# fulliu/lc

Measured on AMD Instinct MI355X. Metric: poses/sec (cov-loss fwd+bwd + weighted PnP), B=256 N=64, 1/2/4/8 MI355X, higher is better.
Workload: dtype f64; 1 GPU; configs[1]: synthetic B=256 N=64 2D-3D correspondences per GPU, HIP weighted-PnP + cov-loss; global_batch=256, n_points=64, launch=graph_region, launch_agreed_by_all_ranks=True

## Files before the change

### lc_amd/csrc/lc_common.h

```cpp
#pragma once
#include <hip/hip_runtime.h>

namespace lc {

#ifndef LC_NT_GRAD_STORES
#define LC_NT_GRAD_STORES 1
#endif
typedef float lc_v4f_t __attribute__((ext_vector_type(4)));
__device__ __forceinline__ void store_stream4(float* q, float a, float b, float c, float d) {
#if LC_NT_GRAD_STORES
    lc_v4f_t r = {a, b, c, d};
    __builtin_nontemporal_store(r, reinterpret_cast<lc_v4f_t*>(q));
#else
    *reinterpret_cast<float4*>(q) = make_float4(a, b, c, d);
#endif
}


constexpr int kWave = 64;

constexpr int kDppQuadXor1 = 0xB1;
constexpr int kDppQuadXor2 = 0x4E;
constexpr int kDppIdentity = 0xE4;
constexpr int kDppRowMirror = 0x140;
constexpr int kDppHalfMirror = 0x141;

template <int CTRL, int BANK_MASK = 0xF>
__device__ __forceinline__ double dpp_mov_f64(double old, double src) {
    const int lo = __builtin_amdgcn_update_dpp(__double2loint(old), __double2loint(src), CTRL, 0xF, BANK_MASK, false);
    const int hi = __builtin_amdgcn_update_dpp(__double2hiint(old), __double2hiint(src), CTRL, 0xF, BANK_MASK, false);
    return __hiloint2double(hi, lo);
}

__device__ __forceinline__ double shfl_f64(double v, int src) {
    const int lo = __shfl(__double2loint(v), src, kWave), hi = __shfl(__double2hiint(v), src, kWave);
    return __hiloint2double(hi, lo);
}

__device__ __forceinline__ double swap32_add(double a, double b) {
    const auto lo = __builtin_amdgcn_permlane32_swap(__double2loint(a), __double2loint(b), false, false);
    const auto hi = __builtin_amdgcn_permlane32_swap(__double2hiint(a), __double2hiint(b), false, false);
    return __hiloint2double(hi[0], lo[0]) + __hiloint2double(hi[1], lo[1]);
}
__device__ __forceinline__ double swap16_add(double a, double b) {
    const auto lo = __builtin_amdgcn_permlane16_swap(__double2loint(a), __double2loint(b), false, false);
    const auto hi = __builtin_amdgcn_permlane16_swap(__double2hiint(a), __double2hiint(b), false, false);
    return __hiloint2double(hi[0], lo[0]) + __hiloint2double(hi[1], lo[1]);
}

template <int CTRL, int BANK_UP>
__device__ __forceinline__ double dpp_exchange_add(double lo, double hi) {
    constexpr int BANK_DOWN = 0xF & ~BANK_UP;
    const double keep = dpp_mov_f64<kDppIdentity, BANK_UP>(lo, hi);
    double recv = dpp_mov_f64<CTRL, BANK_UP>(lo, hi);
    recv = dpp_mov_f64<CTRL, BANK_DOWN>(recv, lo);
    return keep + recv;
}

template <int K>
__device__ __forceinline__ void wave_allreduce(double (&v)[K]) {
#pragma unroll
    for (int i = 0; i < K; ++i) {
        double x = v[i];
        x += dpp_mov_f64<kDppQuadXor1>(x, x);
        x += dpp_mov_f64<kDppQuadXor2>(x, x);
        x += dpp_mov_f64<kDppHalfMirror>(x, x);
        x += dpp_mov_f64<kDppRowMirror>(x, x);
        x = swap16_add(x, x);
        x = swap32_add(x, x);
        v[i] = x;
    }
}

template <int K>
__device__ __forceinline__ void wave_reduce_scatter16(double (&v)[K], int ) {
    static_assert(K % 16 == 0, "K must be a multiple of 16");
    constexpr int R = K / 16;
#pragma unroll
    for (int i = 0; i < K / 2; ++i) v[i] = swap32_add(v[i], v[i + K / 2]);
#pragma unroll
    for (int i = 0; i < K / 4; ++i) v[i] = swap16_add(v[i], v[i + K / 4]);
#pragma unroll
    for (int i = 0; i < K / 8; ++i) v[i] = dpp_exchange_add<kDppRowMirror, 0xC>(v[i], v[i + K / 8]);
#pragma unroll
    for (int i = 0; i < K / 16; ++i) v[i] = dpp_exchange_add<kDppHalfMirror, 0xA>(v[i], v[i + K / 16]);
#pragma unroll
    for (int i = 0; i < R; ++i) {
        v[i] += dpp_mov_f64<kDppQuadXor2>(v[i], v[i]);
        v[i] += dpp_mov_f64<kDppQuadXor1>(v[i], v[i]);
    }
}

__device__ __forceinline__ int scatter16_base(int lane, int R) {
    return R * (((lane >> 5) & 1) * 8 + ((lane >> 4) & 1) * 4 + ((lane >> 3) & 1) * 2 + ((lane >> 2) & 1));
}

__device__ __forceinline__ double fast_rcp(double x) {
    const double y = __builtin_amdgcn_rcp(x);
    const double e = __builtin_fma(-x, y, 1.0);
    return __builtin_fma(y, e, y);
}

__device__ __forceinline__ void fast_sqrt_rsqrt(double x, double& s, double& rs) {
    const double r0 = __builtin_amdgcn_rsq(x);
    const double g = x * r0, h = 0.5 * r0;
    const double rr = __builtin_fma(-h, g, 0.5);
    const double g1 = __builtin_fma(g, rr, g), h1 = __builtin_fma(h, rr, h);
    s = x == 0.0 ? 0.0 : g1;
    rs = x == 0.0 ? r0 : 2.0 * h1;
}
__device__ __forceinline__ double fast_sqrt(double x) {
    double s, rs;
    fast_sqrt_rsqrt(x, s, rs);
    return s;
}

template <int NW>
constexpr int sum_bcast_lds_doubles(int K) { return K * 68 * NW + K; }

#ifndef LC_WAVE_SYNC
#define LC_WAVE_SYNC 0
#endif
__device__ __forceinline__ void wave_sync() {
    __builtin_amdgcn_fence(__ATOMIC_RELEASE, "wavefront");
    __builtin_amdgcn_wave_barrier();
    __builtin_amdgcn_fence(__ATOMIC_ACQUIRE, "wavefront");
}

template <class T>
__device__ __forceinline__ void xcd_store(T* q, T v) { __hip_atomic_store(q, v, __ATOMIC_RELAXED, __HIP_MEMORY_SCOPE_AGENT); }
template <class T>
__device__ __forceinline__ T xcd_load(const T* q) { return __hip_atomic_load(q, __ATOMIC_RELAXED, __HIP_MEMORY_SCOPE_AGENT); }
__device__ __forceinline__ void xcd_stores_done() { asm volatile("s_waitcnt vmcnt(0)" ::: "memory"); }

constexpr int kArrivalShards = 16, kArrivalStride = 32;
constexpr int kArrivalWords = (1 + kArrivalShards) * kArrivalStride;
__device__ __forceinline__ bool arrive_is_last(unsigned* words, unsigned block, unsigned blocks) {
    const unsigned shards = blocks < (unsigned)kArrivalShards ? blocks : (unsigned)kArrivalShards;
    const unsigned g = block % shards, members = (blocks - g + shards - 1) / shards;
    if (__hip_atomic_fetch_add(words + (1 + g) * kArrivalStride, 1u, __ATOMIC_RELAXED, __HIP_MEMORY_SCOPE_AGENT) != members - 1) return false;
    return __hip_atomic_fetch_add(words, 1u, __ATOMIC_RELAXED, __HIP_MEMORY_SCOPE_AGENT) == shards - 1;
}
__device__ __forceinline__ void arrival_reset(unsigned* words, int tid) {
    if (tid <= kArrivalShards) xcd_store(words + tid * kArrivalStride, 0u);
}

template <int NW>
__device__ __forceinline__ void block_sum_sync() {
    if constexpr (NW == 1 && !LC_WAVE_SYNC) wave_sync();
    else __syncthreads();
}

template <int NW>
__device__ __forceinline__ int block_sum_open(int tid) {
    block_sum_sync<NW>();
    return tid + 2 * (tid >> 5);
}
template <int NW>
__device__ __forceinline__ void block_sum_put(double* lds, int pos, int k, double v) { lds[k * (68 * NW) + pos] = v; }

template <int K, int NW>
__device__ __forceinline__ void block_sum_close(double (&v)[K], double* lds, int tid);

template <int K, int NW>
__device__ __forceinline__ void block_sum_bcast_lds(double (&v)[K], double* lds, int tid) {
    const int pos = block_sum_open<NW>(tid);
#pragma unroll
    for (int k = 0; k < K; ++k) block_sum_put<NW>(lds, pos, k, v[k]);
    block_sum_close<K, NW>(v, lds, tid);
}

template <int K, int NW>
__device__ __forceinline__ double* block_sum_totals(double* lds) { return lds + K * (68 * NW); }

template <int K, int NW>
__device__ __forceinline__ void block_sum_reduce(double* lds, int tid) {
    static_assert(K <= 32 && (NW == 1 || NW == 4), "unsupported shape");
    constexpr int LD = 68 * NW, S = 2 * NW;
    block_sum_sync<NW>();
    double s = 0;
    if (tid < K * S) {
        const double2* row = reinterpret_cast<const double2*>(lds + (tid / S) * LD + 34 * (tid % S));
        double2 a[8];
#pragma unroll
        for (int i = 0; i < 8; ++i) a[i] = row[i];
#pragma unroll
        for (int i = 0; i < 8; ++i) {
            const double2 t = row[8 + i];
            a[i].x += t.x;
            a[i].y += t.y;
        }
#pragma unroll
        for (int st = 4; st >= 1; st >>= 1) {
#pragma unroll
            for (int i = 0; i < st; ++i) { a[i].x += a[i + st].x; a[i].y += a[i + st].y; }
        }
        s = a[0].x + a[0].y;
    }
    s += dpp_mov_f64<kDppQuadXor1>(s, s);
    if constexpr (NW == 4) {
        s += dpp_mov_f64<kDppQuadXor2>(s, s);
        s += dpp_mov_f64<kDppHalfMirror>(s, s);
    }
    double* tot = lds + K * LD;
    if (tid < K * S && (tid % S) == 0) tot[tid / S] = s;
    block_sum_sync<NW>();
}

template <int K, int NW>
__device__ __forceinline__ void block_sum_close(double (&v)[K], double* lds, int tid) {
    block_sum_reduce<K, NW>(lds, tid);
    const double* tot = block_sum_totals<K, NW>(lds);
#pragma unroll
    for (int k = 0; k < K; ++k) v[k] = tot[k];
}

#ifndef LC_WIDE_SUM_REGS
#define LC_WIDE_SUM_REGS 1
#endif
template <int K>
__device__ __forceinline__ void block_sum_waves4(double (&v)[K], double* lds, int tid, int& phase) {
    static_assert(K <= 32, "one reduce-scatter of 32");
    const int lane = tid & 63, wave = tid >> 6;
    double w[32];
#pragma unroll
    for (int k = 0; k < 32; ++k) w[k] = k < K ? v[k] : 0.0;
    wave_reduce_scatter16<32>(w, lane);
    double* part = lds;
    double* tot = lds + 128 + 32 * phase;
    phase ^= 1;
    if ((lane & 3) == 0) *reinterpret_cast<double2*>(part + 32 * wave + scatter16_base(lane, 2)) = make_double2(w[0], w[1]);
    __syncthreads();
    if (tid < 32) tot[tid] = ((part[tid] + part[32 + tid]) + part[64 + tid]) + part[96 + tid];
    __syncthreads();
#pragma unroll
    for (int k = 0; k < K; ++k) v[k] = tot[k];
}

constexpr int kSplitMaxParts = 8;
#ifndef LC_SPLIT_WAIT_US
#define LC_SPLIT_WAIT_US 2000
#endif
constexpr unsigned long long kSplitWaitTicks = 100ull * LC_SPLIT_WAIT_US;
__device__ __forceinline__ bool split_wait_expired(int polls, unsigned long long& t0) {
    if ((polls & 15) != 15) return false;
    const unsigned long long now = __builtin_amdgcn_s_memrealtime();
    if (t0 == 0) { t0 = now; return false; }
    return now - t0 > kSplitWaitTicks;
}
constexpr int kSplitRowWords = 64;
constexpr size_t kSplitPoseBytes = 2 * kSplitMaxParts * kSplitRowWords * sizeof(unsigned long long) + 128;
constexpr int kSplitLdsDoubles = 128 + 64 + 2;
constexpr int kSplitSerialLdsDoubles = 128 + 32 * kSplitMaxParts + 32;
struct SplitSum {
    unsigned long long* exch;
    unsigned* epoch;
    int G, part;
    unsigned base;
    unsigned seq;
    bool timed_out;
};
__device__ __forceinline__ unsigned* split_tail(void* region, size_t region_bytes) {
    return reinterpret_cast<unsigned*>(static_cast<char*>(region) + region_bytes - 128);
}
__device__ __forceinline__ SplitSum split_sum_enter(void* pose_region, int G, int part) {
    unsigned* epoch = split_tail(pose_region, kSplitPoseBytes);
    return SplitSum{reinterpret_cast<unsigned long long*>(pose_region), epoch, G, part, xcd_load(epoch), 0u, false};
}
__device__ __forceinline__ void split_sum_leave(const SplitSum& sx) {
    if (sx.timed_out) xcd_store(sx.epoch + 1, 1u);
    else if (sx.part == 0 && sx.seq > 0) xcd_store(sx.epoch, sx.base + sx.seq);
}
__device__ __forceinline__ bool split_rescue_enter(void* region, size_t region_bytes, bool redo, int tid, int threads) {
    unsigned* tail = split_tail(region, region_bytes);
    const bool dirty = xcd_load(tail + 1) != 0u;
    if (!dirty && !redo) return false;
    __syncthreads();
    if (dirty) {
        unsigned long long* w = static_cast<unsigned long long*>(region);
        for (size_t i = tid; i < (region_bytes - 128) / 8; i += threads) xcd_store(w + i, 0ull);
        if (tid < 2) xcd_store(tail + tid, 0u);
    }
    if (redo && tid == 0) xcd_store(tail + 2, xcd_load(tail + 2) + 1u);
    return redo;
}

template <int K>
__device__ __forceinline__ void block_sum_split(double (&v)[K], double* lds, int tid, int& phase, SplitSum& sx) {
    static_assert(K <= 32, "one reduce-scatter of 32");
    const int lane = tid & 63, wave = tid >> 6;
    double w[32];
#pragma unroll
    for (int k = 0; k < 32; ++k) w[k] = k < K ? v[k] : 0.0;
    wave_reduce_scatter16<32>(w, lane);
    double* part = lds;
    double* tot = lds + 128 + 32 * phase;
    int* arrived_ok = reinterpret_cast<int*>(lds + 192);
    phase ^= 1;
    if (sx.timed_out) {
#pragma unroll
        for (int k = 0; k < K; ++k) v[k] = 0.0;
        return;
    }
    if ((lane & 3) == 0) *reinterpret_cast<double2*>(part + 32 * wave + scatter16_base(lane, 2)) = make_double2(w[0], w[1]);
    __syncthreads();
    if (tid < 32) {
        const unsigned long long ticket = (unsigned long long)(sx.base + sx.seq + 1u) << 32;
        unsigned long long* rows = sx.exch + (size_t)(sx.seq & 1u) * (kSplitMaxParts * kSplitRowWords) + 2 * tid;
        {
            const unsigned long long bits = __builtin_bit_cast(unsigned long long, ((part[tid] + part[32 + tid]) + part[64 + tid]) + part[96 + tid]);
            unsigned long long* mine = rows + sx.part * kSplitRowWords;
            xcd_store(mine, ticket | (bits & 0xFFFFFFFFull));
            xcd_store(mine + 1, ticket | (bits >> 32));
        }
        unsigned long long lo[kSplitMaxParts], hi[kSplitMaxParts];
        bool ok = true;
        unsigned long long t0 = 0;
        for (int polls = 0;; ++polls) {
#pragma unroll
            for (int g = 0; g < kSplitMaxParts; ++g)
                if (g < sx.G) {
                    lo[g] = xcd_load(rows + g * kSplitRowWords);
                    hi[g] = xcd_load(rows + g * kSplitRowWords + 1);
                }
            unsigned long long late = 0;
#pragma unroll
            for (int g = 0; g < kSplitMaxParts; ++g)
                if (g < sx.G) late |= ((lo[g] ^ ticket) | (hi[g] ^ ticket)) >> 32;
            if (late == 0) break;
            if (split_wait_expired(polls, t0)) { ok = false; break; }
            __builtin_amdgcn_s_sleep(1);
        }
        double s = 0.0;
#pragma unroll
        for (int g = 0; g < kSplitMaxParts; ++g)
            if (g < sx.G) s += __builtin_bit_cast(double, (hi[g] << 32) | (lo[g] & 0xFFFFFFFFull));
        tot[tid] = s;
        if (!ok) *arrived_ok = 0;
    }
    __syncthreads();
    if (!*arrived_ok) sx.timed_out = true;
#pragma unroll
    for (int k = 0; k < K; ++k) v[k] = tot[k];
    ++sx.seq;
}

template <int K>
__device__ __forceinline__ void block_sum_parts_serial(double (&v)[K], double* lds, int tid, int g, int G) {
    static_assert(K <= 32, "one reduce-scatter of 32");
    const int lane = tid & 63, wave = tid >> 6;
    double w[32];
#pragma unroll
    for (int k = 0; k < 32; ++k) w[k] = k < K ? v[k] : 0.0;
    wave_reduce_scatter16<32>(w, lane);
    double* part = lds;
    double* rows = lds + 128;
    double* tot = lds + 128 + 32 * kSplitMaxParts;
    if ((lane & 3) == 0) *reinterpret_cast<double2*>(part + 32 * wave + scatter16_base(lane, 2)) = make_double2(w[0], w[1]);
    __syncthreads();
    if (tid < 32) {
        rows[32 * g + tid] = ((part[tid] + part[32 + tid]) + part[64 + tid]) + part[96 + tid];
        if (g == G - 1) {
            double s = 0.0;
            for (int h = 0; h < G; ++h) s += rows[32 * h + tid];
            tot[tid] = s;
        }
    }
    __syncthreads();
    if (g == G - 1) {
#pragma unroll
        for (int k = 0; k < K; ++k) v[k] = tot[k];
    }
}

#ifndef LC_HORNER_ASM
#define LC_HORNER_ASM 1
#endif
__device__ __forceinline__ double horner_step(double p, double z, double c) {
#if LC_HORNER_ASM
    double r;
    asm("v_fma_f64 %0, %1, %2, %3" : "=v"(r) : "v"(p), "v"(z), "v"(c));
    return r;
#else
    return __builtin_fma(p, z, c);
#endif
}

__device__ __forceinline__ void sincos_small(double x, double& s, double& c) {
    if (!(x < 1.0e4)) {
        sincos(x, &s, &c);
        return;
    }
    const double kf = __builtin_rint(x * 0.63661977236758134308);
    const int q = (int)kf;
    double r = __builtin_fma(-kf, 1.57079632673412561417e+00, x);
    r = __builtin_fma(-kf, 6.07710050650619224932e-11, r);
    r = __builtin_fma(-kf, 2.02226624879595063154e-21, r);
    const double z = r * r;
    double ps = horner_step(1.58969099521155010221e-10, z, -2.50507602534068634195e-08);
    ps = horner_step(ps, z, 2.75573137070700676789e-06);
    ps = horner_step(ps, z, -1.98412698298579493134e-04);
    ps = horner_step(ps, z, 8.33333333332248946124e-03);
    ps = horner_step(ps, z, -1.66666666666666324348e-01);
    const double sr = __builtin_fma(ps * z, r, r);
    double pc = horner_step(-1.13596475577881948265e-11, z, 2.08757232129817482790e-09);
    pc = horner_step(pc, z, -2.75573143513906633035e-07);
    pc = horner_step(pc, z, 2.48015872894767294178e-05);
    pc = horner_step(pc, z, -1.38888888888741095749e-03);
    pc = horner_step(pc, z, 4.16666666666666019037e-02);
    const double cr = __builtin_fma(pc * z, z, __builtin_fma(-0.5, z, 1.0));
    const double ss = (q & 1) ? cr : sr, cc = (q & 1) ? sr : cr;
    s = (q & 2) ? -ss : ss;
    c = ((q + 1) & 2) ? -cc : cc;
}

__device__ __forceinline__ double atan_ratio_pos(double s, double c) {
    const bool swap = s > c;
    const double a = swap ? c : s, b = swap ? s : c;
    double t = a * fast_rcp(b);
#pragma unroll
    for (int k = 0; k < 2; ++k) {
        const double h = fast_sqrt(__builtin_fma(t, t, 1.0));
        t = t * fast_rcp(1.0 + h);
    }
    const double w = t * t;
    double p = horner_step(-1.0 / 21.0, w, 1.0 / 19.0);
    p = horner_step(p, w, -1.0 / 17.0);
    p = horner_step(p, w, 1.0 / 15.0);
    p = horner_step(p, w, -1.0 / 13.0);
    p = horner_step(p, w, 1.0 / 11.0);
    p = horner_step(p, w, -1.0 / 9.0);
    p = horner_step(p, w, 1.0 / 7.0);
    p = horner_step(p, w, -1.0 / 5.0);
    p = horner_step(p, w, 1.0 / 3.0);
    const double at = 4.0 * __builtin_fma(-(p * w), t, t);
    return swap ? 1.57079632679489661923 - at : at;
}

__device__ __forceinline__ bool uniform(bool c) { return __builtin_amdgcn_ballot_w64(c) != 0ull; }

__host__ __device__ constexpr int tri6(int i, int j) { return i * 6 - (i * (i - 1)) / 2 + (j - i); }

}
```

### lc_amd/csrc/lc_pnp_body.h

```cpp
#pragma once
#include <cfloat>

#include "lc_common.h"
#include "lc_kernels.h"

#ifdef LC_STAMPS
#define LC_PSTAMP_DECL unsigned long long pst_[8] = {0, 0, 0, 0, 0, 0, 0, 0}, pt0_ = 0, pt1_ = 0
#define LC_PSTAMP_BEGIN()                                                                 \
    do {                                                                                  \
        __builtin_amdgcn_sched_barrier(0);                                                \
        asm volatile("s_memtime %0\n\ts_waitcnt lgkmcnt(0)" : "=s"(pt0_)::"memory");      \
        __builtin_amdgcn_sched_barrier(0);                                                \
    } while (0)
#define LC_PSTAMP(i)                                                                      \
    do {                                                                                  \
        __builtin_amdgcn_sched_barrier(0);                                                \
        asm volatile("s_memtime %0\n\ts_waitcnt lgkmcnt(0)" : "=s"(pt1_)::"memory");      \
        __builtin_amdgcn_sched_barrier(0);                                                \
        pst_[i] += pt1_ - pt0_;                                                           \
        pt0_ = pt1_;                                                                      \
    } while (0)
#else
#define LC_PSTAMP_DECL
#define LC_PSTAMP_BEGIN() do {} while (0)
#define LC_PSTAMP(i) do {} while (0)
#endif

#ifndef LC_WIDE_REG_SUM_REGS
#define LC_WIDE_REG_SUM_REGS 1
#endif
#ifndef LC_PNP_STREAM_SUM
#define LC_PNP_STREAM_SUM 1
#endif

namespace lc {
namespace pnp {

template <int NW>
constexpr int kPnpLdsDoubles = sum_bcast_lds_doubles<NW>(28);

struct Point {
    double X[3];
    double u, v;
    double a, b, c;
};

struct Rot {
    double R[9];
    double Jr[9];
};

__device__ __forceinline__ void make_rot(const double aa[3], Rot& o) {
    const double x = aa[0], y = aa[1], z = aa[2];
    const double th2 = x * x + y * y + z * z;
    const bool small = !(th2 > DBL_EPSILON);
    double th, ith;
    fast_sqrt_rsqrt(th2, th, ith);
    double s, c;
    sincos_small(th, s, c);
    const double ith2 = ith * ith;
    const double A = small ? 1.0 : s * ith;
    const double B = small ? 0.0 : (1.0 - c) * ith2;
    const double C = small ? 0.0 : (th - s) * ith2 * ith;
    const double cd = small ? 1.0 : c;
    o.R[0] = cd + B * x * x;    o.R[1] = B * x * y - A * z; o.R[2] = B * x * z + A * y;
    o.R[3] = B * x * y + A * z; o.R[4] = cd + B * y * y;    o.R[5] = B * y * z - A * x;
    o.R[6] = B * x * z - A * y; o.R[7] = B * y * z + A * x; o.R[8] = cd + B * z * z;
    const double d = 1.0 - C * th2;
    o.Jr[0] = d + C * x * x;     o.Jr[1] = C * x * y + B * z; o.Jr[2] = C * x * z - B * y;
    o.Jr[3] = C * x * y - B * z; o.Jr[4] = d + C * y * y;     o.Jr[5] = C * y * z + B * x;
    o.Jr[6] = C * x * z + B * y; o.Jr[7] = C * y * z - B * x; o.Jr[8] = d + C * z * z;
}

template <bool FIRST, bool STREAM = false, int NW = 1>
__device__ __forceinline__ void accumulate_point(const Point& pt, const Rot& rt, const double t[3], const double k[6],
                                                 const double (&sc)[6], double (&acc)[28], double* lds = nullptr, int pos = 0) {
    double rx[3], q[3];
#pragma unroll
    for (int d = 0; d < 3; ++d) {
        rx[d] = rt.R[3 * d] * pt.X[0] + rt.R[3 * d + 1] * pt.X[1] + rt.R[3 * d + 2] * pt.X[2];
        q[d] = rx[d] + t[d];
    }
    const double iz = fast_rcp(q[2]);
    const double up = (q[0] * k[0] + q[1] * k[1]) * iz, vp = (q[0] * k[3] + q[1] * k[4]) * iz;
    const double du = up - pt.u, dv = vp - pt.v;
    const double r[2] = {du * pt.a + dv * pt.b, dv * pt.c};
    const double dup[3] = {k[0] * iz, k[1] * iz, -up * iz};
    const double dvp[3] = {k[3] * iz, k[4] * iz, -vp * iz};
    double J[2][6];
#pragma unroll
    for (int m = 0; m < 3; ++m) {
        J[0][3 + m] = pt.a * dup[m] + pt.b * dvp[m];
        J[1][3 + m] = pt.c * dvp[m];
    }
#pragma unroll
    for (int rr = 0; rr < 2; ++rr) {
        double cr[3];
        cr[0] = rx[1] * J[rr][5] - rx[2] * J[rr][4];
        cr[1] = rx[2] * J[rr][3] - rx[0] * J[rr][5];
        cr[2] = rx[0] * J[rr][4] - rx[1] * J[rr][3];
#pragma unroll
        for (int m = 0; m < 3; ++m) J[rr][m] = (rt.Jr[3 * m] * cr[0] + rt.Jr[3 * m + 1] * cr[1] + rt.Jr[3 * m + 2] * cr[2]) * sc[m];
#pragma unroll
        for (int m = 0; m < 3; ++m) J[rr][3 + m] *= sc[3 + m];
    }
#pragma unroll
    for (int i = 0; i < 6; ++i) {
#pragma unroll
        for (int j = i; j < 6; ++j) {
            const double v = __builtin_fma(J[0][i], J[0][j], J[1][i] * J[1][j]);
            if constexpr (STREAM) block_sum_put<NW>(lds, pos, tri6(i, j), v);
            else acc[tri6(i, j)] = FIRST ? v : acc[tri6(i, j)] + v;
        }
        const double gi = __builtin_fma(J[0][i], r[0], J[1][i] * r[1]);
        if constexpr (STREAM) block_sum_put<NW>(lds, pos, 21 + i, gi);
        else acc[21 + i] = FIRST ? gi : acc[21 + i] + gi;
    }
    const double ss = __builtin_fma(r[0], r[0], r[1] * r[1]);
    if constexpr (STREAM) block_sum_put<NW>(lds, pos, 27, ss);
    else acc[27] = FIRST ? ss : acc[27] + ss;
}

__device__ __forceinline__ bool ldlt_solve6(const double (&A)[21], const double (&dg)[6], const double (&rhs)[6], double (&y)[6]) {
    double L[6][6], Ld[6][6], id[6];
    bool ok = true;
#pragma unroll
    for (int j = 0; j < 6; ++j) {
        double dj = A[tri6(j, j)] + dg[j];
#pragma unroll
        for (int k = 0; k < j; ++k) dj -= L[j][k] * Ld[j][k];
        ok = ok && (dj > 0) && (dj < DBL_MAX);
        id[j] = fast_rcp(dj);
#pragma unroll
        for (int i = j + 1; i < 6; ++i) {
            double v = A[tri6(j, i)];
#pragma unroll
            for (int k = 0; k < j; ++k) v -= L[i][k] * Ld[j][k];
            Ld[i][j] = v;
            L[i][j] = v * id[j];
        }
    }
    double z[6];
#pragma unroll
    for (int i = 0; i < 6; ++i) {
        double v = rhs[i];
#pragma unroll
        for (int k = 0; k < i; ++k) v -= L[i][k] * z[k];
        z[i] = v;
    }
#pragma unroll
    for (int i = 5; i >= 0; --i) {
        double v = z[i] * id[i];
#pragma unroll
        for (int k = i + 1; k < 6; ++k) v -= L[k][i] * y[k];
        y[i] = v;
    }
    return ok;
}

struct RawPoint {
    float X[3];
    float2 u;
    float a, b, c;
};
__device__ __forceinline__ float nan_to_num(float f) { return f != f ? 0.f : fminf(fmaxf(f, -FLT_MAX), FLT_MAX); }

template <bool OPTS = false>
__device__ __forceinline__ RawPoint load_raw_point(const PnpParams& p, size_t base, int n) {
    RawPoint o;
    const float* X = p.pts3d + (base + n) * 3;
    o.u = *reinterpret_cast<const float2*>(p.pts2d + (base + n) * 2);
    o.X[0] = X[0]; o.X[1] = X[1]; o.X[2] = X[2];
    if (OPTS && p.weight_mask) {
        const float m = p.weight_mask[base + n] ? 1.f : 0.f;
        o.a = m; o.b = 0.f; o.c = m;
    } else if (p.sqrtL) {
        const float4 L = *reinterpret_cast<const float4*>(p.sqrtL + (base + n) * 4);
        o.a = L.x; o.b = L.z; o.c = L.w;
    } else {
        const float2 L = *reinterpret_cast<const float2*>(p.sqrt_diag + (base + n) * 2);
        o.a = L.x; o.b = 0.f; o.c = L.y;
    }
    if constexpr (OPTS) {
        if (p.options & kPnpWeightsAreStd) { o.a = 1.f / (o.a * o.a); o.c = 1.f / (o.c * o.c); }
        if (p.options & kPnpNanToNum) {
            o.u.x = nan_to_num(o.u.x); o.u.y = nan_to_num(o.u.y);
            o.X[0] = nan_to_num(o.X[0]); o.X[1] = nan_to_num(o.X[1]); o.X[2] = nan_to_num(o.X[2]);
            o.a = nan_to_num(o.a); o.b = nan_to_num(o.b); o.c = nan_to_num(o.c);
        }
        if (p.options & kPnpWeightsAreIcov) { o.a = sqrtf(o.a); o.c = sqrtf(o.c); }
    }
    return o;
}
__device__ __forceinline__ Point to_point(const RawPoint& r, const double cam[6]) {
    Point o;
    o.X[0] = r.X[0]; o.X[1] = r.X[1]; o.X[2] = r.X[2];
    o.u = (double)r.u.x - cam[2];
    o.v = (double)r.u.y - cam[5];
    o.a = r.a; o.b = r.b; o.c = r.c;
    return o;
}
template <bool OPTS = false>
__device__ __forceinline__ Point load_point(const PnpParams& p, size_t base, int n, const double cam[6]) {
    return to_point(load_raw_point<OPTS>(p, base, n), cam);
}

__device__ __forceinline__ double max_abs6(const double (&v)[6]) {
    double m = 0;
#pragma unroll
    for (int j = 0; j < 6; ++j) m = fmax(m, fabs(v[j]));
    return m;
}
__device__ __forceinline__ double norm6(const double (&v)[6]) {
    double m = 0;
#pragma unroll
    for (int j = 0; j < 6; ++j) m += v[j] * v[j];
    return fast_sqrt(m);
}

template <bool REG, int NW = 1, bool TRACE = false, bool OPTS = false, int PPT = 0, bool TAIL = false, int SPLIT = 0>
__device__ __forceinline__ void solve_pose(const PnpParams& p, int b, int lane, double* bc, bool store = true, float* handoff = nullptr,
                                           const float* start_override = nullptr, [[maybe_unused]] SplitSum* sx = nullptr) {
    constexpr int kThreads = kWave * NW;
    static_assert(SPLIT != 1 || (NW == 4 && !REG && PPT > 0 && !TRACE), "the split form is the four-wave cached-prefix solve");
    static_assert(SPLIT != 2 || (NW == 4 && !REG && PPT == 0 && !TRACE), "the rescue form walks memory, part by part");
    const int slot = SPLIT == 1 ? lane + kThreads * sx->part : lane;
    const int stride = SPLIT == 1 ? kThreads * sx->G : kThreads;
#ifdef LC_TRACE_CLOCK
    const unsigned long long t_start_ = __builtin_amdgcn_s_memtime();
#endif
    LC_PSTAMP_DECL;
    LC_PSTAMP_BEGIN();
    const int n = p.counts ? p.counts[b] : p.Nmax;
    const int bk = (OPTS && p.pose_mod > 0) ? b % p.pose_mod : b;
    const float* st_in = start_override ? start_override : (p.start ? p.start + 7 * (size_t)bk : p.states + 7 * (size_t)b);
    const bool filter = OPTS && (p.options & kPnpNanToNum);
    auto fin = [&](float f) { return filter ? nan_to_num(f) : f; };
    if (n < 3) {
        if (lane == 0 && store) {
            p.rets[b] = 1;
            p.result_tr[b] = 1.f;
            if (p.iters) p.iters[b] = 0;
        }
        if (lane < 7) {
            const float v = fin(st_in[lane]);
            if (store && (p.start || start_override || filter)) p.states[7 * (size_t)b + lane] = v;
            if (handoff) handoff[lane] = v;
        }
        return;
    }
    const size_t base = (size_t)b * p.Nmax;
    const bool active = lane < n;
    RawPoint raw;
    if constexpr (REG) raw = load_raw_point<OPTS>(p, base, active ? lane : 0);
    [[maybe_unused]] RawPoint rawc[PPT > 0 ? PPT : 1];
    if constexpr (!REG && PPT > 0) {
#pragma unroll
        for (int k = 0; k < PPT; ++k)
            if (slot + k * stride < n) rawc[k] = load_raw_point<OPTS>(p, base, slot + k * stride);
    }
    double cam[6];
    {
        const float* Kp = p.K + 9 * (size_t)bk;
#pragma unroll
        for (int i = 0; i < 6; ++i) cam[i] = fin(Kp[i]);
    }
    double x[6];
    {
        float stf[7];
#pragma unroll
        for (int i = 0; i < 7; ++i) stf[i] = st_in[i];
        asm volatile("" : "+v"(stf[0]), "+v"(stf[1]), "+v"(stf[2]), "+v"(stf[3]), "+v"(stf[4]), "+v"(stf[5]), "+v"(stf[6]));
        const double q0 = fin(stf[0]), q1 = fin(stf[1]), q2 = fin(stf[2]), q3 = fin(stf[3]);
        const double s2 = q1 * q1 + q2 * q2 + q3 * q3;
        double kk = 2.0;
        if (s2 > 0.0) {
            const double s = fast_sqrt(s2);
            const double half = atan_ratio_pos(s, fabs(q0));
            const double two_theta = 2.0 * ((q0 < 0.0) ? -half : half);
            kk = two_theta / s;
        }
        x[0] = q1 * kk; x[1] = q2 * kk; x[2] = q3 * kk;
        x[3] = fin(stf[4]); x[4] = fin(stf[5]); x[5] = fin(stf[6]);
    }
    LC_PSTAMP(0);
    Point rp;
    if constexpr (REG) {
        rp = to_point(raw, cam);
        if (!active) { rp.a = 0.0; rp.b = 0.0; rp.c = 0.0; }
    }

    [[maybe_unused]] int sum_phase = 0;
    auto evaluate = [&](const double (&xe)[6], const double (&sc)[6], double (&H)[21], double (&g)[6], double& cost) -> bool {
        LC_PSTAMP(1);
        Rot rt;
        make_rot(xe, rt);
        LC_PSTAMP(2);
        const double t[3] = {xe[3], xe[4], xe[5]};
        double acc[28];
        if constexpr (REG && LC_PNP_STREAM_SUM && !(NW == 4 && LC_WIDE_REG_SUM_REGS)) {
            const int pos = block_sum_open<NW>(lane);
            accumulate_point<true, true, NW>(rp, rt, t, cam, sc, acc, bc, pos);
            LC_PSTAMP(3);
            block_sum_close<28, NW>(acc, bc, lane);
        } else if constexpr (REG) {
            accumulate_point<true>(rp, rt, t, cam, sc, acc);
            LC_PSTAMP(3);
            if constexpr (NW == 4 && LC_WIDE_SUM_REGS) block_sum_waves4<28>(acc, bc, lane, sum_phase);
            else block_sum_bcast_lds<28, NW>(acc, bc, lane);
        } else {
#pragma unroll
            for (int i = 0; i < 28; ++i) acc[i] = 0;
            if constexpr (PPT > 0) {
#pragma unroll
                for (int k = 0; k < PPT; ++k)
                    if (slot + k * stride < n) accumulate_point<false>(to_point(rawc[k], cam), rt, t, cam, sc, acc);
                if constexpr (TAIL)
                    for (int i = slot + PPT * stride; i < n; i += stride) accumulate_point<false>(load_point<OPTS>(p, base, i, cam), rt, t, cam, sc, acc);
            } else if constexpr (SPLIT == 2) {
                for (int g = 0; g < sx->G; ++g) {
                    if (g > 0) {
#pragma unroll
                        for (int i = 0; i < 28; ++i) acc[i] = 0;
                    }
                    for (int i = lane + kThreads * g; i < n; i += kThreads * sx->G) accumulate_point<false>(load_point<OPTS>(p, base, i, cam), rt, t, cam, sc, acc);
                    block_sum_parts_serial<28>(acc, bc, lane, g, sx->G);
                }
            } else {
                for (int i = lane; i < n; i += kThreads) accumulate_point<false>(load_point<OPTS>(p, base, i, cam), rt, t, cam, sc, acc);
            }
            LC_PSTAMP(3);
            if constexpr (SPLIT == 2) {}
            else if constexpr (SPLIT == 1) block_sum_split<28>(acc, bc, lane, sum_phase, *sx);
            else if constexpr (NW == 4 && LC_WIDE_SUM_REGS) block_sum_waves4<28>(acc, bc, lane, sum_phase);
            else block_sum_bcast_lds<28, NW>(acc, bc, lane);
        }
        LC_PSTAMP(4);
#pragma unroll
        for (int i = 0; i < 21; ++i) H[i] = acc[i];
#pragma unroll
        for (int i = 0; i < 6; ++i) g[i] = acc[21 + i];
        const double ss = acc[27];
        cost = 0.5 * ss;
        double chk = ss;
#pragma unroll
        for (int i = 0; i < 6; ++i) chk += H[tri6(i, i)];
        LC_PSTAMP(5);
        if constexpr (SPLIT == 1) {
            if (sx->timed_out) return false;
        }
        return chk <= DBL_MAX;
    };

    const double ftol = p.ftol, ptol = 1e-8, gtol = 1e-10;
    double H[21], g[6], cost;
    double scale[6], iscale[6];
    bool failed;
    {
        const double one[6] = {1, 1, 1, 1, 1, 1};
        failed = !evaluate(x, one, H, g, cost);
#pragma unroll
        for (int j = 0; j < 6; ++j) {
            iscale[j] = 1.0 + fast_sqrt(H[tri6(j, j)]);
            scale[j] = fast_rcp(iscale[j]);
        }
#pragma unroll
        for (int i = 0; i < 6; ++i) {
#pragma unroll
            for (int j = i; j < 6; ++j) H[tri6(i, j)] *= scale[i] * scale[j];
            g[i] *= scale[i];
        }
    }
    auto grad_max = [&](const double (&gs)[6]) {
        double m = 0;
#pragma unroll
        for (int j = 0; j < 6; ++j) m = fmax(m, fabs(gs[j]) * iscale[j]);
        return m;
    };
    double gmax = grad_max(g);
    auto sqnorm6 = [](const double (&v)[6]) {
        double m = 0;
#pragma unroll
        for (int j = 0; j < 6; ++j) m += v[j] * v[j];
        return m;
    };
    double xn2 = sqnorm6(x);
    double radius = 1e4, dfac = 2.0;
    int iter = 0, n_invalid = 0;
    bool converged = false;
    auto trace = [&](int kind, double cost_x, double cost_cand, double mcc, double rho, double step_norm) {
        if constexpr (TRACE) {
            if (lane == 0 && p.trace && iter <= p.trace_rows) {
                double* row = p.trace + ((size_t)b * p.trace_rows + (iter - 1)) * 8;
                row[0] = kind; row[1] = cost_x; row[2] = cost_cand; row[3] = mcc; row[4] = rho; row[5] = step_norm;
                row[6] = radius; row[7] = gmax;
#ifdef LC_TRACE_CLOCK
                row[7] = (double)(__builtin_amdgcn_s_memtime() - t_start_);
#endif
            }
        }
    };

    while (uniform(!failed && !converged)) {
        if (iter >= p.max_iter) break;
        if (uniform(gmax <= gtol || radius <= 1e-32)) { converged = true; break; }
        ++iter;
        double dg[6], y[6];
        const double inv_radius = fast_rcp(radius);
#pragma unroll
        for (int i = 0; i < 6; ++i) dg[i] = fmin(fmax(H[tri6(i, i)], 1e-6), 1e32) * inv_radius;
        LC_PSTAMP(1);
        bool step_ok = ldlt_solve6(H, dg, g, y);
        LC_PSTAMP(6);
        double mcc = 0;
#pragma unroll
        for (int i = 0; i < 6; ++i) mcc += y[i] * (g[i] + dg[i] * y[i]);
        mcc *= 0.5;
        step_ok = step_ok && (mcc > 0.0) && (mcc <= DBL_MAX);
        if (uniform(!step_ok)) {
            if (++n_invalid >= 5) { failed = true; trace(0, cost, 0.0, mcc, 0.0, 0.0); break; }
            radius /= dfac; dfac *= 2.0;
            trace(0, cost, 0.0, mcc, 0.0, 0.0);
            continue;
        }
        n_invalid = 0;
        double xc[6], delta[6];
#pragma unroll
        for (int j = 0; j < 6; ++j) { delta[j] = -y[j] * scale[j]; xc[j] = x[j] + delta[j]; }
        const double sn2 = sqnorm6(delta);
        const bool ptol_in_reach = TRACE || uniform(!(sn2 > 2.0 * ptol * ptol * (xn2 + ptol * ptol)));
        double step_norm = 0.0;
        bool ptol_hit = false;
        if (ptol_in_reach) {
            step_norm = fast_sqrt(sn2);
            ptol_hit = uniform(step_norm <= ptol * (fast_sqrt(xn2) + ptol));
        }
        double cost_c;
        const bool cand_ok = evaluate(xc, scale, H, g, cost_c);
        if constexpr (SPLIT == 1) {
            if (sx->timed_out) { failed = true; break; }
        }
        if (!cand_ok) cost_c = DBL_MAX;
        if (ptol_hit) {
            converged = true; trace(3, cost, cost_c, mcc, 0.0, step_norm); break;
        }
        const double cost_change = cost - cost_c;
        if (uniform(fabs(cost_change) <= ftol * cost)) {
            converged = true; trace(4, cost, cost_c, mcc, cost_change * fast_rcp(mcc), step_norm); break;
        }
        const double rel = cost_change * fast_rcp(mcc);
        if (uniform(rel > 1e-3)) {
#pragma unroll
            for (int j = 0; j < 6; ++j) x[j] = xc[j];
            const double cost_prev = cost;
            cost = cost_c;
            xn2 = sqnorm6(x);
            gmax = grad_max(g);
            const double tq = 2.0 * rel - 1.0;
            radius = fmin(1e16, radius * fast_rcp(fmax(1.0 / 3.0, 1.0 - tq * tq * tq)));
            dfac = 2.0;
            trace(1, cost_prev, cost_c, mcc, rel, step_norm);
        } else {
            radius /= dfac; dfac *= 2.0;
            trace(2, cost, cost_c, mcc, rel, step_norm);
            double cost_again;
            if (!evaluate(x, scale, H, g, cost_again)) { failed = true; break; }
        }
    }
    LC_PSTAMP(1);
#ifdef LC_STAMPS
    if (lane == 0 && p.iters) {
        unsigned long long* o = reinterpret_cast<unsigned long long*>(p.iters) + 8 * (size_t)b;
        for (int i = 0; i < 6; ++i) o[i] = pst_[i];
        o[6] = iter;
        o[7] = pst_[6];
    }
#endif
    const bool invalid = failed || !converged;
    if (invalid && lane < 7) {
        const float v = fin(st_in[lane]);
        if (store && (p.start || start_override || filter)) p.states[7 * (size_t)b + lane] = v;
        if (handoff) handoff[lane] = v;
    }
    if (lane == 0) {
        if (store) {
            p.rets[b] = invalid ? 1 : 0;
            if constexpr (SPLIT == 1) {
                if (sx->timed_out) p.rets[b] = kPnpPartNeverArrived;
            }
            p.result_tr[b] = (float)radius;
#ifndef LC_STAMPS
            if (p.iters) p.iters[b] = iter;
#endif
        }
        if (!invalid) {
            float stq[7];
            float* st = stq;
            const double t2 = x[0] * x[0] + x[1] * x[1] + x[2] * x[2];
            double q0 = 1.0, kk = 0.5;
            if (t2 > 0.0) {
                const double th = fast_sqrt(t2), h = 0.5 * th;
                double sh, ch;
                sincos_small(h, sh, ch);
                q0 = ch;
                kk = sh / th;
            }
            st[0] = (float)q0; st[1] = (float)(x[0] * kk); st[2] = (float)(x[1] * kk); st[3] = (float)(x[2] * kk);
            st[4] = (float)x[3]; st[5] = (float)x[4]; st[6] = (float)x[5];
#pragma unroll
            for (int k = 0; k < 7; ++k) {
                if (store) p.states[7 * (size_t)b + k] = stq[k];
                if (handoff) handoff[k] = stq[k];
            }
        }
    }
}


constexpr int kPnpLowregLdsDoubles = kPnpLdsDoubles<1> + 30;

__device__ __forceinline__ bool ldlt_solve6_lds(const double* A, const double* g, double inv_radius, double (&y)[6], double& mcc) {
    double L[6][6], Ld[6][6], id[6];
    bool ok = true;
    auto dgv = [&](int i) { return fmin(fmax(A[tri6(i, i)], 1e-6), 1e32) * inv_radius; };
#pragma unroll
    for (int j = 0; j < 6; ++j) {
        double dj = A[tri6(j, j)] + dgv(j);
#pragma unroll
        for (int k = 0; k < j; ++k) dj -= L[j][k] * Ld[j][k];
        ok = ok && (dj > 0) && (dj < DBL_MAX);
        id[j] = fast_rcp(dj);
#pragma unroll
        for (int i = j + 1; i < 6; ++i) {
            double v = A[tri6(j, i)];
#pragma unroll
            for (int k = 0; k < j; ++k) v -= L[i][k] * Ld[j][k];
            Ld[i][j] = v;
            L[i][j] = v * id[j];
        }
    }
    double z[6];
#pragma unroll
    for (int i = 0; i < 6; ++i) {
        double v = g[i];
#pragma unroll
        for (int k = 0; k < i; ++k) v -= L[i][k] * z[k];
        z[i] = v;
    }
#pragma unroll
    for (int i = 5; i >= 0; --i) {
        double v = z[i] * id[i];
#pragma unroll
        for (int k = i + 1; k < 6; ++k) v -= L[k][i] * y[k];
        y[i] = v;
    }
    mcc = 0;
#pragma unroll
    for (int i = 0; i < 6; ++i) mcc += y[i] * (g[i] + dgv(i) * y[i]);
    mcc *= 0.5;
    return ok;
}

template <bool OPTS = false>
__device__ __forceinline__ void solve_pose_lowreg(const PnpParams& p, int b, int lane, double* bc) {
    const int n = p.counts ? p.counts[b] : p.Nmax;
    const int bk = (OPTS && p.pose_mod > 0) ? b % p.pose_mod : b;
    const float* st_in = (p.start ? p.start + 7 * (size_t)bk : p.states + 7 * (size_t)b);
    const bool filter = OPTS && (p.options & kPnpNanToNum);
    auto fin = [&](float f) { return filter ? nan_to_num(f) : f; };
    if (n < 3) {
        if (lane == 0) {
            p.rets[b] = 1;
            p.result_tr[b] = 1.f;
            if (p.iters) p.iters[b] = 0;
        }
        if ((p.start || filter) && lane < 7) p.states[7 * (size_t)b + lane] = fin(st_in[lane]);
        return;
    }
    const size_t base = (size_t)b * p.Nmax;
    const bool active = lane < n;
    const RawPoint raw = load_raw_point<OPTS>(p, base, active ? lane : 0);
    double cam[6];
    {
        const float* Kp = p.K + 9 * (size_t)bk;
#pragma unroll
        for (int i = 0; i < 6; ++i) cam[i] = fin(Kp[i]);
    }
    double* const tot = block_sum_totals<28, 1>(bc);
    double* const ux = bc + kPnpLdsDoubles<1>;
    double* const uscale = ux + 6;
    double* const uiscale = ux + 12;
    double* const uxc = ux + 18;
    double* const ucam = ux + 24;
    if (lane == 0) {
#pragma unroll
        for (int i = 0; i < 6; ++i) ucam[i] = cam[i];
    }
    {
        double x[6];
        const double q0 = fin(st_in[0]), q1 = fin(st_in[1]), q2 = fin(st_in[2]), q3 = fin(st_in[3]);
        const double s2 = q1 * q1 + q2 * q2 + q3 * q3;
        double kk = 2.0;
        if (s2 > 0.0) {
            const double s = fast_sqrt(s2);
            const double half = atan_ratio_pos(s, fabs(q0));
            const double two_theta = 2.0 * ((q0 < 0.0) ? -half : half);
            kk = two_theta / s;
        }
        x[0] = q1 * kk; x[1] = q2 * kk; x[2] = q3 * kk;
        x[3] = fin(st_in[4]); x[4] = fin(st_in[5]); x[5] = fin(st_in[6]);
        if (lane == 0) {
#pragma unroll
            for (int j = 0; j < 6; ++j) { ux[j] = x[j]; uscale[j] = 1.0; }
        }
        wave_sync();
    }
    Point rp = to_point(raw, cam);
    if (!active) { rp.a = 0.0; rp.b = 0.0; rp.c = 0.0; }

    auto evaluate = [&](const double* xe, double& cost) -> bool {
        double xv[6], sc[6];
#pragma unroll
        for (int j = 0; j < 6; ++j) { xv[j] = xe[j]; sc[j] = uscale[j]; }
        Rot rt;
        make_rot(xv, rt);
        const double t[3] = {xv[3], xv[4], xv[5]};
        double acc[28];
        const int pos = block_sum_open<1>(lane);
        accumulate_point<true, true, 1>(rp, rt, t, ucam, sc, acc, bc, pos);
        block_sum_reduce<28, 1>(bc, lane);
        const double ss = tot[27];
        cost = 0.5 * ss;
        double chk = ss;
#pragma unroll
        for (int i = 0; i < 6; ++i) chk += tot[tri6(i, i)];
        return chk <= DBL_MAX;
    };

    const double ftol = p.ftol, ptol = 1e-8, gtol = 1e-10;
    double cost;
    bool failed = !evaluate(ux, cost);
    {
        double scale[6], iscale[6];
#pragma unroll
        for (int j = 0; j < 6; ++j) {
            iscale[j] = 1.0 + fast_sqrt(tot[tri6(j, j)]);
            scale[j] = fast_rcp(iscale[j]);
        }
        double Hs[21], gs[6];
#pragma unroll
        for (int i = 0; i < 6; ++i) {
#pragma unroll
            for (int j = i; j < 6; ++j) { double h = tot[tri6(i, j)]; h *= scale[i] * scale[j]; Hs[tri6(i, j)] = h; }
            double gi = tot[21 + i]; gi *= scale[i]; gs[i] = gi;
        }
        wave_sync();
        if (lane == 0) {
#pragma unroll
            for (int k = 0; k < 21; ++k) tot[k] = Hs[k];
#pragma unroll
            for (int j = 0; j < 6; ++j) { tot[21 + j] = gs[j]; uscale[j] = scale[j]; uiscale[j] = iscale[j]; }
        }
        wave_sync();
    }
    auto grad_max = [&]() {
        double m = 0;
#pragma unroll
        for (int j = 0; j < 6; ++j) m = fmax(m, fabs(tot[21 + j]) * uiscale[j]);
        return m;
    };
    auto sqnorm6 = [](const double* v) {
        double m = 0;
#pragma unroll
        for (int j = 0; j < 6; ++j) m += v[j] * v[j];
        return m;
    };
    double gmax = grad_max();
    double xn2 = sqnorm6(ux);
    double radius = 1e4, dfac = 2.0;
    int iter = 0, n_invalid = 0;
    bool converged = false;

    while (uniform(!failed && !converged)) {
        if (iter >= p.max_iter) break;
        if (uniform(gmax <= gtol || radius <= 1e-32)) { converged = true; break; }
        ++iter;
        double y[6], mcc;
        const double inv_radius = fast_rcp(radius);
        bool step_ok = ldlt_solve6_lds(tot, tot + 21, inv_radius, y, mcc);
        step_ok = step_ok && (mcc > 0.0) && (mcc <= DBL_MAX);
        if (uniform(!step_ok)) {
            if (++n_invalid >= 5) { failed = true; break; }
            radius /= dfac; dfac *= 2.0;
            continue;
        }
        n_invalid = 0;
        double sn2;
        {
            double xc[6], delta[6];
#pragma unroll
            for (int j = 0; j < 6; ++j) { delta[j] = -y[j] * uscale[j]; xc[j] = ux[j] + delta[j]; }
            sn2 = 0;
#pragma unroll
            for (int j = 0; j < 6; ++j) sn2 += delta[j] * delta[j];
            if (lane == 0) {
#pragma unroll
                for (int j = 0; j < 6; ++j) uxc[j] = xc[j];
            }
            wave_sync();
        }
        const bool ptol_in_reach = uniform(!(sn2 > 2.0 * ptol * ptol * (xn2 + ptol * ptol)));
        bool ptol_hit = false;
        if (ptol_in_reach) ptol_hit = uniform(fast_sqrt(sn2) <= ptol * (fast_sqrt(xn2) + ptol));
        double cost_c;
        const bool cand_ok = evaluate(uxc, cost_c);
        if (!cand_ok) cost_c = DBL_MAX;
        if (ptol_hit) { converged = true; break; }
        const double cost_change = cost - cost_c;
        if (uniform(fabs(cost_change) <= ftol * cost)) { converged = true; break; }
        const double rel = cost_change * fast_rcp(mcc);
        if (uniform(rel > 1e-3)) {
            double xn[6];
#pragma unroll
            for (int j = 0; j < 6; ++j) xn[j] = uxc[j];
            wave_sync();
            if (lane == 0) {
#pragma unroll
                for (int j = 0; j < 6; ++j) ux[j] = xn[j];
            }
            wave_sync();
            cost = cost_c;
            xn2 = sqnorm6(ux);
            gmax = grad_max();
            const double tq = 2.0 * rel - 1.0;
            radius = fmin(1e16, radius * fast_rcp(fmax(1.0 / 3.0, 1.0 - tq * tq * tq)));
            dfac = 2.0;
        } else {
            radius /= dfac; dfac *= 2.0;
            double cost_again;
            if (!evaluate(ux, cost_again)) { failed = true; break; }
        }
    }
    const bool invalid = failed || !converged;
    if (invalid && (p.start || filter) && lane < 7) p.states[7 * (size_t)b + lane] = fin(st_in[lane]);
    if (lane == 0) {
        p.rets[b] = invalid ? 1 : 0;
        p.result_tr[b] = (float)radius;
        if (p.iters) p.iters[b] = iter;
        if (!invalid) {
            float* st = p.states + 7 * (size_t)b;
            double x[6];
#pragma unroll
            for (int j = 0; j < 6; ++j) x[j] = ux[j];
            const double t2 = x[0] * x[0] + x[1] * x[1] + x[2] * x[2];
            double q0 = 1.0, kk = 0.5;
            if (t2 > 0.0) {
                const double th = fast_sqrt(t2), h = 0.5 * th;
                double sh, ch;
                sincos_small(h, sh, ch);
                q0 = ch;
                kk = sh / th;
            }
            st[0] = (float)q0; st[1] = (float)(x[0] * kk); st[2] = (float)(x[1] * kk); st[3] = (float)(x[2] * kk);
            st[4] = (float)x[3]; st[5] = (float)x[4]; st[6] = (float)x[5];
        }
    }
}

}
}
```

Measured before the change: 19.79 million poses/s.

## Add cost-only evaluation shortcut for terminal LM iterations in weighted PnP

Adds a cheap cost-only evaluation path (rotation without Jacobian, projection, single-row block reduction) used when the predicted cost change is small enough that the ftol convergence test is likely to fire. This skips the full Hessian/gradient accumulation and 28-way reduction on the final iteration. It also exits early on ptol before any evaluation. It adds an extra bounds check meant to mirror the full evaluate's finiteness test, and reads ftol as float, which may slightly change termination behavior. When the shortcut does not fire, the extra cost evaluation is wasted work.

Result: slower. 18.76 million poses/s (-5.2%).

```diff
diff --git a/lc_amd/csrc/lc_common.h b/lc_amd/csrc/lc_common.h
--- a/lc_amd/csrc/lc_common.h
+++ b/lc_amd/csrc/lc_common.h
@@ -173,38 +173,49 @@
 template <int K, int NW>
 __device__ __forceinline__ double* block_sum_totals(double* lds) { return lds + K * (68 * NW); }
 
+__device__ __forceinline__ double block_sum_segment(const double2* row) {
+    double2 a[8];
+#pragma unroll
+    for (int i = 0; i < 8; ++i) a[i] = row[i];
+#pragma unroll
+    for (int i = 0; i < 8; ++i) {
+        const double2 t = row[8 + i];
+        a[i].x += t.x;
+        a[i].y += t.y;
+    }
+#pragma unroll
+    for (int st = 4; st >= 1; st >>= 1) {
+#pragma unroll
+        for (int i = 0; i < st; ++i) { a[i].x += a[i + st].x; a[i].y += a[i + st].y; }
+    }
+    return a[0].x + a[0].y;
+}
+
 template <int K, int NW>
 __device__ __forceinline__ void block_sum_reduce(double* lds, int tid) {
     static_assert(K <= 32 && (NW == 1 || NW == 4), "unsupported shape");
     constexpr int LD = 68 * NW, S = 2 * NW;
     block_sum_sync<NW>();
     double s = 0;
-    if (tid < K * S) {
-        const double2* row = reinterpret_cast<const double2*>(lds + (tid / S) * LD + 34 * (tid % S));
-        double2 a[8];
-#pragma unroll
-        for (int i = 0; i < 8; ++i) a[i] = row[i];
-#pragma unroll
-        for (int i = 0; i < 8; ++i) {
-            const double2 t = row[8 + i];
-            a[i].x += t.x;
-            a[i].y += t.y;
-        }
-#pragma unroll
-        for (int st = 4; st >= 1; st >>= 1) {
-#pragma unroll
-            for (int i = 0; i < st; ++i) { a[i].x += a[i + st].x; a[i].y += a[i + st].y; }
-        }
-        s = a[0].x + a[0].y;
-    }
+    if (tid < K * S) s = block_sum_segment(reinterpret_cast<const double2*>(lds + (tid / S) * LD + 34 * (tid % S)));
     s += dpp_mov_f64<kDppQuadXor1>(s, s);
     if constexpr (NW == 4) {
         s += dpp_mov_f64<kDppQuadXor2>(s, s);
         s += dpp_mov_f64<kDppHalfMirror>(s, s);
     }
     double* tot = lds + K * LD;
+    if constexpr (NW == 1) asm volatile("" : "+v"(tid));
     if (tid < K * S && (tid % S) == 0) tot[tid / S] = s;
     block_sum_sync<NW>();
+}
+
+template <int ROW>
+__device__ __forceinline__ double block_sum_reduce_row(const double* lds, int tid) {
+    block_sum_sync<1>();
+    asm volatile("" : "+v"(tid));
+    double s = block_sum_segment(reinterpret_cast<const double2*>(lds + ROW * 68 + 34 * (tid & 1)));
+    s += dpp_mov_f64<kDppQuadXor1>(s, s);
+    return s;
 }
 
 template <int K, int NW>
diff --git a/lc_amd/csrc/lc_pnp_body.h b/lc_amd/csrc/lc_pnp_body.h
--- a/lc_amd/csrc/lc_pnp_body.h
+++ b/lc_amd/csrc/lc_pnp_body.h
@@ -50,6 +50,7 @@
     double Jr[9];
 };
 
+template <bool JR = true>
 __device__ __forceinline__ void make_rot(const double aa[3], Rot& o) {
     const double x = aa[0], y = aa[1], z = aa[2];
     const double th2 = x * x + y * y + z * z;
@@ -66,25 +67,36 @@
     o.R[0] = cd + B * x * x;    o.R[1] = B * x * y - A * z; o.R[2] = B * x * z + A * y;
     o.R[3] = B * x * y + A * z; o.R[4] = cd + B * y * y;    o.R[5] = B * y * z - A * x;
     o.R[6] = B * x * z - A * y; o.R[7] = B * y * z + A * x; o.R[8] = cd + B * z * z;
-    const double d = 1.0 - C * th2;
-    o.Jr[0] = d + C * x * x;     o.Jr[1] = C * x * y + B * z; o.Jr[2] = C * x * z - B * y;
-    o.Jr[3] = C * x * y - B * z; o.Jr[4] = d + C * y * y;     o.Jr[5] = C * y * z + B * x;
-    o.Jr[6] = C * x * z + B * y; o.Jr[7] = C * y * z - B * x; o.Jr[8] = d + C * z * z;
-}
+    if constexpr (JR) {
+        const double d = 1.0 - C * th2;
+        o.Jr[0] = d + C * x * x;     o.Jr[1] = C * x * y + B * z; o.Jr[2] = C * x * z - B * y;
+        o.Jr[3] = C * x * y - B * z; o.Jr[4] = d + C * y * y;     o.Jr[5] = C * y * z + B * x;
+        o.Jr[6] = C * x * z + B * y; o.Jr[7] = C * y * z - B * x; o.Jr[8] = d + C * z * z;
+    }
+}
+
+__device__ __forceinline__ void project_point(const Point& pt, const double (&R)[9], const double t[3], const double k[6], double (&rx)[3],
+                                              double& iz, double& up, double& vp, double (&r)[2]) {
+    double q[3];
+#pragma unroll
+    for (int d = 0; d < 3; ++d) {
+        rx[d] = R[3 * d] * pt.X[0] + R[3 * d + 1] * pt.X[1] + R[3 * d + 2] * pt.X[2];
+        q[d] = rx[d] + t[d];
+    }
+    iz = fast_rcp(q[2]);
+    up = (q[0] * k[0] + q[1] * k[1]) * iz;
+    vp = (q[0] * k[3] + q[1] * k[4]) * iz;
+    const double du = up - pt.u, dv = vp - pt.v;
+    r[0] = du * pt.a + dv * pt.b;
+    r[1] = dv * pt.c;
+}
+__device__ __forceinline__ double residual_sq(const double (&r)[2]) { return __builtin_fma(r[0], r[0], r[1] * r[1]); }
 
 template <bool FIRST, bool STREAM = false, int NW = 1>
 __device__ __forceinline__ void accumulate_point(const Point& pt, const Rot& rt, const double t[3], const double k[6],
                                                  const double (&sc)[6], double (&acc)[28], double* lds = nullptr, int pos = 0) {
-    double rx[3], q[3];
-#pragma unroll
-    for (int d = 0; d < 3; ++d) {
-        rx[d] = rt.R[3 * d] * pt.X[0] + rt.R[3 * d + 1] * pt.X[1] + rt.R[3 * d + 2] * pt.X[2];
-        q[d] = rx[d] + t[d];
-    }
-    const double iz = fast_rcp(q[2]);
-    const double up = (q[0] * k[0] + q[1] * k[1]) * iz, vp = (q[0] * k[3] + q[1] * k[4]) * iz;
-    const double du = up - pt.u, dv = vp - pt.v;
-    const double r[2] = {du * pt.a + dv * pt.b, dv * pt.c};
+    double rx[3], iz, up, vp, r[2];
+    project_point(pt, rt.R, t, k, rx, iz, up, vp, r);
     const double dup[3] = {k[0] * iz, k[1] * iz, -up * iz};
     const double dvp[3] = {k[3] * iz, k[4] * iz, -vp * iz};
     double J[2][6];
@@ -116,7 +128,7 @@
         if constexpr (STREAM) block_sum_put<NW>(lds, pos, 21 + i, gi);
         else acc[21 + i] = FIRST ? gi : acc[21 + i] + gi;
     }
-    const double ss = __builtin_fma(r[0], r[0], r[1] * r[1]);
+    const double ss = residual_sq(r);
     if constexpr (STREAM) block_sum_put<NW>(lds, pos, 27, ss);
     else acc[27] = FIRST ? ss : acc[27] + ss;
 }
@@ -352,7 +364,33 @@
         return chk <= DBL_MAX;
     };
 
+    constexpr bool kTerminalShortcut = REG && NW == 1 && !TRACE && SPLIT == 0;
+    [[maybe_unused]] auto evaluate_cost = [&](const double (&xe)[6], double& cost) -> bool {
+        Rot rt;
+        make_rot<false>(xe, rt);
+        const double t[3] = {xe[3], xe[4], xe[5]};
+        double rx[3], iz, up, vp, r[2];
+        project_point(rp, rt.R, t, cam, rx, iz, up, vp, r);
+        const int pos = block_sum_open<1>(lane);
+        block_sum_put<1>(bc, pos, 27, residual_sq(r));
+        double a0 = rp.a, k0 = cam[0];
+        asm volatile("" : "+v"(a0), "+v"(k0));
+        const double kk = ((fabs(k0) + fabs(cam[1])) + fabs(cam[3])) + fabs(cam[4]);
+        const double jr = 3.0 + ((fabs(xe[0]) + fabs(xe[1])) + fabs(xe[2]));
+        const double m = ((fabs(a0) + fabs(rp.b)) + fabs(rp.c)) * fabs(iz) * (kk + (fabs(up) + fabs(vp))) *
+                         ((1.0 + (fabs(rx[0]) + fabs(rx[1]))) + fabs(rx[2])) * jr;
+        const bool bounded = !uniform(!(m <= 1e100));
+        const double ss = block_sum_reduce_row<27>(bc, lane);
+        cost = 0.5 * ss;
+        return bounded && ss <= DBL_MAX;
+    };
+
     const double ftol = p.ftol, ptol = 1e-8, gtol = 1e-10;
+    [[maybe_unused]] auto ftol_now = [&]() -> double {
+        float f = p.ftol;
+        asm volatile("" : "+s"(f));
+        return f;
+    };
     double H[21], g[6], cost;
     double scale[6], iscale[6];
     bool failed;
@@ -435,6 +473,17 @@
             step_norm = fast_sqrt(sn2);
             ptol_hit = uniform(step_norm <= ptol * (fast_sqrt(xn2) + ptol));
         }
+        if constexpr (kTerminalShortcut) {
+            constexpr double kPredictC = 1.25;
+            if (ptol_hit) { converged = true; break; }
+            double cost_o = cost;
+            asm volatile("" : "+v"(cost_o));
+            const double ftol_cost = ftol_now() * cost_o;
+            if (uniform(mcc <= kPredictC * ftol_cost)) {
+                double cost_t;
+                if (evaluate_cost(xc, cost_t) && uniform(fabs(cost - cost_t) <= ftol_cost)) { converged = true; break; }
+            }
+        }
         double cost_c;
         const bool cand_ok = evaluate(xc, scale, H, g, cost_c);
         if constexpr (SPLIT == 1) {
@@ -445,7 +494,7 @@
             converged = true; trace(3, cost, cost_c, mcc, 0.0, step_norm); break;
         }
         const double cost_change = cost - cost_c;
-        if (uniform(fabs(cost_change) <= ftol * cost)) {
+        if (uniform(fabs(cost_change) <= (kTerminalShortcut ? ftol_now() : ftol) * cost)) {
             converged = true; trace(4, cost, cost_c, mcc, cost_change * fast_rcp(mcc), step_norm); break;
         }
         const double rel = cost_change * fast_rcp(mcc);
```
